# angelvillar96/STLPose

Hardware: AMD Instinct MI355X
Metric: images/sec/GPU HRNet-W32 384x288 train step; PCKh@0.5 parity (higher is better)
Workload: dtype f16/bf16; 1 GPU; HRNet-W32 384x288 bs=32/GPU train step (fwd+MSE+bwd+Adam), random-init weights; global_batch=32, parallelism=dp1

## Files before the change

stlpose_amd/csrc/conv1x1.inc:

```
template <typename T, int G, bool Q, int OCC, typename TY = T, int EO = -1, bool ZM = false>
__global__ __launch_bounds__(512, OCC) void conv1x1_kernel(const ConvK k) {
    extern __shared__ __attribute__((aligned(16))) char smem[];
    constexpr int NTHR = 512, WM = 4, MT = 4, NTW = 2, BCO = 64, TPX = 256;
    constexpr int KV = ET<T>::KV, CK = ET<T>::CK;
    constexpr int PSG = G * 64 + 32;
    constexpr int VPP = 4 * G;
    constexpr int RPT = NTHR / VPP;
    constexpr int NVA = TPX / RPT;
    constexpr int NVB = BCO / RPT;
    constexpr int GK = G * CK;
    static_assert(NVB >= 1, "filter staging needs at least one vector per thread");
    const stl_conv& p = k.p;
    const int tid = threadIdx.x, lane = tid & 63, wave = tid >> 6, r16 = lane & 15, g = lane >> 4;
    const int wm = wave % WM, wn = wave / WM;
    const int bl = blockIdx.x >> 3;
    const int by = bl % k.ny, lx = bl / k.ny;
    const int n0 = by * BCO;
    const int xcd = blockIdx.x & 7, nx = (gridDim.x >> 3) / k.ny;
    const int P = p.B * p.Ho * p.Wo;

    float* cs = reinterpret_cast<float*>(smem + k.off_cs);
    float* cm = reinterpret_cast<float*>(smem + k.off_cm);
    char* sA = smem + k.off_a;
    char* sB = smem + k.off_b;

    for (int c = tid; c < k.cipad; c += NTHR) {
        float a = 0.f, b = 0.f, cc = 0.f;
        if (c < p.Ci) src_consts(p.src, c, p.Ci, a, b, cc);
        cs[c] = a, cs[k.cipad + c] = b, cs[2 * k.cipad + c] = cc;
    }
    if (p.mask_y) {
        for (int c = tid; c < BCO; c += NTHR) {
            float a = 0.f, b = 0.f, mu = 0.f, rs = 0.f;
            if (n0 + c < p.Co) {
                bn_mean_rstd(p.mask_bn, n0 + c, p.Co, mu, rs);
                bn_affine(p.mask_bn.gamma[n0 + c], p.mask_bn.beta[n0 + c], mu, rs, a, b);
            }
            cm[c] = a, cm[BCO + c] = b, cm[2 * BCO + c] = mu, cm[3 * BCO + c] = rs;
        }
    }

    const int a_part = tid % VPP, a_row = tid / VPP;
    V16 ra[NVA], rq[Q ? NVA : 1], rb[NVB];

    auto issue = [&](int P0, int k0, bool en) {
        const int ch = k0 + a_part * KV;
        const bool chok = en && ch < p.Ci;
#pragma unroll
        for (int i = 0; i < NVA; ++i) {
            const int pix = P0 + a_row + i * RPT;
            const size_t off = (chok && pix < P) ? (size_t)pix * p.Ci + ch : 0;
            ra[i] = ldg16((const char*)p.src.x + off * sizeof(T));
            if (Q) rq[i] = ldg16((const char*)p.src.y + off * sizeof(T));
        }
        if (!k.wres) {
#pragma unroll
            for (int i = 0; i < NVB; ++i) {
                const int n = n0 + a_row + i * RPT;
                const size_t off = (chok && n < p.Co) ? (size_t)n * p.Ci + ch : 0;
                rb[i] = ldg16((const char*)p.w + off * sizeof(T));
            }
        }
    };
    const float relu_lo = p.src.relu ? 0.f : -INFINITY;
    auto write_lds = [&](int P0, int k0) {
        const int ch = k0 + a_part * KV;
        const bool chok = ch < p.Ci;
        const int chc = chok ? ch : 0;
#pragma unroll
        for (int i = 0; i < NVA; ++i) {
            const bool ok = chok && (P0 + a_row + i * RPT) < P;
            V16 val = ra[i];
            if constexpr (ZM) {
                val = xform_bnadd<T>(val, rq[i], cs + chc, cs + k.cipad + chc, relu_lo);
                if (ok && by == 0 && p.src_out) stg16((char*)p.src_out + ((size_t)(P0 + a_row + i * RPT) * p.Ci + ch) * sizeof(T), val);
            } else if (Q)
                val = xform_bnbwd<T, TY>(val, rq[i], cs + chc, cs + k.cipad + chc, cs + 2 * k.cipad + chc);
            else if (p.src.mode != STL_SRC_PLAIN)
                val = xform_bn<T>(val, cs + chc, cs + k.cipad + chc, relu_lo);
            mask16(val, ok);
            *reinterpret_cast<V16*>(sA + (a_row + i * RPT) * PSG + a_part * 16) = val;
        }
        if (!k.wres) {
#pragma unroll
            for (int i = 0; i < NVB; ++i) {
                V16 val = rb[i];
                mask16(val, chok && (n0 + a_row + i * RPT) < p.Co);
                *reinterpret_cast<V16*>(sB + (a_row + i * RPT) * PSG + a_part * 16) = val;
            }
        }
    };

    if (k.wres) {
        const bool chok = a_part * KV < p.Ci;
#pragma unroll
        for (int i = 0; i < NVB; ++i) {
            const int n = n0 + a_row + i * RPT;
            const size_t off = (chok && n < p.Co) ? (size_t)n * p.Ci + a_part * KV : 0;
            rb[i] = ldg16((const char*)p.w + off * sizeof(T));
        }
    }

    f2v s0[NTW][2], s1[NTW][2];
#pragma unroll
    for (int ni = 0; ni < NTW; ++ni)
#pragma unroll
        for (int h = 0; h < 2; ++h) s0[ni][h] = f2v{0.f, 0.f}, s1[ni][h] = f2v{0.f, 0.f};
    f32x4 acc[MT][NTW];
#pragma unroll
    for (int mi = 0; mi < MT; ++mi)
#pragma unroll
        for (int ni = 0; ni < NTW; ++ni) acc[mi][ni] = f32x4{0.f, 0.f, 0.f, 0.f};

    int xoff[MT];
#pragma unroll
    for (int mi = 0; mi < MT; ++mi) xoff[mi] = ((wm * MT + mi) * 16 + r16) * PSG + g * 16;
    const int woff = (wn * NTW * 16 + r16) * PSG + g * 16;

    const int T8 = (k.npt + 7) >> 3;
    int it = lx, t = xcd * T8 + it, ch0 = 0;
    bool have = (it < T8) && (t < k.npt);
    issue(t * TPX, 0, have);
    if (k.wres) {
        const bool chok = a_part * KV < p.Ci;
#pragma unroll
        for (int i = 0; i < NVB; ++i) {
            V16 val = rb[i];
            mask16(val, chok && (n0 + a_row + i * RPT) < p.Co);
            *reinterpret_cast<V16*>(sB + (a_row + i * RPT) * PSG + a_part * 16) = val;
        }
    }
    __syncthreads();

    while (have) {
        const int P0 = t * TPX;
        write_lds(P0, ch0 * GK);
        __syncthreads();
        const bool last_chunk = (ch0 + 1 == k.nchunks);
        int itn = it, tn = t, chn = ch0 + 1;
        bool have_n = true;
        if (last_chunk) {
            itn = it + nx, tn = xcd * T8 + itn, chn = 0;
            have_n = (itn < T8) && (tn < k.npt);
        }
        issue(tn * TPX, chn * GK, have_n);
#pragma unroll
        for (int sub = 0; sub < G; ++sub) {
            V16 wf[NTW], xf[MT];
#pragma unroll
            for (int ni = 0; ni < NTW; ++ni) wf[ni] = *reinterpret_cast<const V16*>(sB + woff + ni * 16 * PSG + sub * 64);
#pragma unroll
            for (int mi = 0; mi < MT; ++mi) xf[mi] = *reinterpret_cast<const V16*>(sA + xoff[mi] + sub * 64);
#pragma unroll
            for (int mi = 0; mi < MT; ++mi)
#pragma unroll
                for (int ni = 0; ni < NTW; ++ni) mma16<T>(acc[mi][ni], wf[ni], xf[mi]);
        }
        __syncthreads();
        if (last_chunk) {
#pragma unroll
            for (int mi = 0; mi < MT; ++mi) {
                const int pix = P0 + (wm * MT + mi) * 16 + r16;
                const bool pok = pix < P;
                epilogue_tile<T, NTW, BCO, false, TY, EO>(p, acc[mi], cm, pok, pok ? (size_t)pix * p.Co : 0, n0, wn * NTW * 16, g, s0, s1);
            }
        }
        it = itn, t = tn, ch0 = chn, have = have_n;
    }
    double* dst = p.out_stats ? p.out_stats : p.red;
    if (dst) {
        xor_reduce_stats<NTW>(s0, s1);
        float* red = reinterpret_cast<float*>(smem + k.off_red);
        __syncthreads();
        if (r16 == 0) {
#pragma unroll
            for (int ni = 0; ni < NTW; ++ni)
#pragma unroll
                for (int r = 0; r < 4; ++r) {
                    const int cl = (wn * NTW + ni) * 16 + 4 * g + r;
                    red[(wm * 2 + 0) * BCO + cl] = s0[ni][r >> 1][r & 1];
                    red[(wm * 2 + 1) * BCO + cl] = s1[ni][r >> 1][r & 1];
                }
        }
        __syncthreads();
        for (int e = tid; e < 2 * BCO; e += NTHR) {
            const int which = e / BCO, cl = e - which * BCO;
            float s = 0.f;
#pragma unroll
            for (int w = 0; w < WM; ++w) s += red[(w * 2 + which) * BCO + cl];
            if (n0 + cl < p.Co)
                atomicAdd(dst + (size_t)(blockIdx.x & (STL_NSHARD - 1)) * 2 * p.Co + which * p.Co + n0 + cl, (double)s);
        }
    }
}

template <typename T, typename TY, int G, bool Q, int OCC, int EO = -1, bool ZM = false>
int launch_1x1(const ConvK& k, dim3 grid, size_t lds, hipStream_t st) {
    static bool attr_done = false;
    if (!attr_done) {
        (void)hipFuncSetAttribute(reinterpret_cast<const void*>(&conv1x1_kernel<T, G, Q, OCC, TY, EO, ZM>), hipFuncAttributeMaxDynamicSharedMemorySize,
                                  160 * 1024);
        attr_done = true;
    }
    STL_LAUNCH((conv1x1_kernel<T, G, Q, OCC, TY, EO, ZM>), grid, dim3(512), lds, st, k);
    static char nbuf[160];
    static const char* nm = stl_kname<T>(nbuf, "conv1x1_kernel", {G, Q, OCC, stl_code<TY>(), EO, ZM});
    stl_note_kernel(nm, true);
    STL_LAUNCH_CHECK("conv1x1");
    return 0;
}

static bool use_1x1(const stl_conv& p) { return p.ks == 1 && p.stride == 1 && !p.stuff && p.Ci >= 64 && p.Co >= 64; }

template <typename T, typename TY>
int run_1x1(const stl_conv& p, hipStream_t st) {
    constexpr int CK = ET<T>::CK;
    constexpr int G = 2;
    const int gk = G * CK, psg = G * 64 + 32;
    ConvK k;
    memset(&k, 0, sizeof(k));
    k.p = p;
    k.nchunks = ceil_div(p.Ci, gk);
    k.cipad = k.nchunks * gk;
    k.wres = k.nchunks == 1;
    int off = 3 * k.cipad * 4;
    k.off_cs = 0, k.off_cm = off;
    off += 4 * 64 * 4;
    off = (off + 15) & ~15;
    k.off_a = off;
    off += 256 * psg;
    k.off_b = off;
    off += 64 * psg;
    k.off_red = k.off_a;
    const size_t lds = (size_t)off;
    const int P = p.B * p.Ho * p.Wo;
    k.npt = ceil_div(P, 256);
    k.ny = ceil_div(p.Co, 64);
    int gx = ceil_div(k.npt, 8) * 8;
    int cap = std::max(8, (512 / k.ny + 7) / 8 * 8);
    if (const char* e = getenv("STL_CONV_GRID_CAP")) cap = atoi(e) > 0 ? (atoi(e) + 7) / 8 * 8 : cap;
    if (gx > cap) gx = cap;
    dim3 grid(gx * k.ny, 1);
    if (getenv("STL_CONV_DEBUG"))
        fprintf(stderr, "[stl conv1x1] %dx%d Ci%d Co%d: G=%d npt=%d grid=(%d x %d) lds=%zu nchunks=%d\n", p.Ho, p.Wo, p.Ci, p.Co, G, k.npt, gx,
                k.ny, lds, k.nchunks);
    if (p.src.mode == STL_SRC_BNADD) {
        if constexpr (std::is_same<T, TY>::value) {
            const int eoz = epi_code(p);
            if (eoz == 8) return launch_1x1<T, T, 2, true, 4, 8, true>(k, grid, lds, st);
            if (eoz == 0) return launch_1x1<T, T, 2, true, 4, 0, true>(k, grid, lds, st);
        }
        return stl_set_error("conv1x1: a BNADD source takes no epilogue operands");
    }
    const bool q = p.src.mode == STL_SRC_BNBWD;
    const char* noeo = getenv("STL_CONV_NO_EO");
    const int eo = (noeo && (atoi(noeo) & 2)) ? -1 : epi_code(p);
    if (q) {
        if constexpr (!stl_fwd_only<T>) {
            if (eo == 2) return launch_1x1<T, TY, 2, true, 4, 2>(k, grid, lds, st);
            return launch_1x1<T, TY, 2, true, 4>(k, grid, lds, st);
        }
    }
    if constexpr (std::is_same<T, TY>::value) {
        if (eo == 8) return launch_1x1<T, T, 2, false, 4, 8>(k, grid, lds, st);
        return launch_1x1<T, T, 2, false, 4>(k, grid, lds, st);
    }
    return stl_set_error("conv1x1: no kernel for this dtype combination");
}
```

stlpose_amd/csrc/conv_core.hip:

```cpp
#include <stdlib.h>
#include <algorithm>
#include <cstring>
#include <type_traits>
#include "common.cuh"

#ifndef STL_DT
#define STL_DT 2
#endif
#define STL_HAS_F32 (STL_DT == 0 || STL_DT == 2)
#define STL_HAS_BF16 (STL_DT == 1 || STL_DT == 2)
#define STL_HAS_F16 (STL_DT == 3 || STL_DT == 2)
#define STL_HAS_F32S (STL_DT == 4 || STL_DT == 2)

struct ConvK {
    stl_conv p;
    int tiles_c, npt;
    int HR, HC, HP;
    int PI, pad, seff;
    int nchunks, wres;
    int cipad;
    int off_cs, off_cm, off_a, off_b, off_red;
    int sz_a, sz_b;
    int TH, TW;
    int dbg;
// ... 242 lines not shown
    const int T8 = (k.npt + 7) >> 3;
    const int vpitch = p.Ho + 1;

    int it_n = lx, t_n = xcd * T8 + lx, ch_n = 0;
    bool have_n = (it_n < T8) && (t_n < k.npt);
    auto prefetch = [&]() __attribute__((always_inline)) {
        if (have_n && ch_n == 0) tile_setup(t_n, a_go);
        st_t = t_n, st_ch = ch_n, st_have = have_n;
        issue(a_go, ch_n * CK, have_n);
        if (++ch_n == k.nchunks) {
            ch_n = 0, it_n += nx, t_n = xcd * T8 + it_n;
            have_n = have_n && (it_n < T8) && (t_n < k.npt);
        }
    };
    STAMP(3);
    if constexpr (!DB) {
        prefetch();
        if (wres) {
#pragma unroll
            for (int i = 0; i < NVB; ++i) {
                const bool ok = b_g[i] >= 0 && (((tid + i * NTHR) & 3) * KV) < p.Ci;
                V16 val = rb[i];
                mask16(val, ok);
                if (tid + i * NTHR < BCO * TAPS * 4) *reinterpret_cast<V16*>(sB + b_l[i]) = val;
            }
        }
        __syncthreads();
    }
    STAMP(4);

    f32x4 acc[MT][NTW];
#pragma unroll
    for (int mi = 0; mi < MT; ++mi)
#pragma unroll
        for (int ni = 0; ni < NTW; ++ni) acc[mi][ni] = f32x4{0.f, 0.f, 0.f, 0.f};

    constexpr bool EPRE = (OCC <= 1 && WM == 4 && WN == 2 && NTW == 2) && Q && !PE && !ZM && sizeof(T) == 2;
    constexpr bool EBURST = !EPRE && (EO == 1 || EO == 2) && !PE && sizeof(T) == 2;
    auto out_pixel = [&](int vr0, int c0, int mi, bool& pok) __attribute__((always_inline)) -> size_t {
        const int eb0 = sdiv(vr0, k.m_vp), ey0 = vr0 - eb0 * vpitch;
        int eyx = e_yx[mi];
        if constexpr (DB) {
            const int m = (wm * MT + mi) * 16 + r16, ty_ = fdiv(m, k.r_TW);
            eyx = m < tilepx ? ((ty_ << 16) | (m - ty_ * k.TW)) : -1;
        }
        const int ty = eyx >> 16, tx = eyx & 0xffff;
        const int oy0 = ey0 + ty, c = c0 + tx;
        const int wr_ = fdiv(oy0, k.r_vp);
        const int oy = mad24_vsv(wr_, -vpitch, oy0), b = eb0 + wr_;
        pok = (eyx >= 0) & (b < p.B) & (oy < p.Ho) & (c < p.Wo);
        const int e = mulu24_vs(madu24_vsv(madu24_vsv(b, p.Ho, oy), p.Wo, c), p.Co);
        return pok ? (size_t)(uint32_t)e : 0;
    };
    auto epi_fetch = [&](int vr0, int c0, bool* pokv, size_t* pixv, EpiRaw<NTW>* er) __attribute__((always_inline)) {
#pragma unroll
        for (int mi = 0; mi < MT; ++mi) {
            pixv[mi] = out_pixel(vr0, c0, mi, pokv[mi]);
            epilogue_fetch<T, NTW, true, EO>(p, pokv[mi], pixv[mi], n0, wn * NTW * 16, g, er[mi]);
        }
    };

    if constexpr (DB) {
        constexpr int NSLOT = NVA + NVB;
        prefetch();
        int cu_t = st_t, cu_ch = st_ch;
        bool cu_have = st_have;
        __syncthreads();
        write_lds(a_go, st_ch * CK);
        prefetch();
        __syncthreads();
        int img = 0;
        [[maybe_unused]] int dbg_it = 0;
        while (cu_have) {
            STAMP2(4 * dbg_it);
            const int t = cu_t, ch0 = cu_ch;
            const int tr = sdiv(t, k.m_tc), tc = t - tr * k.tiles_c;
            const int vr0 = tr * k.TH, c0 = tc * k.TW;
            const bool last_chunk = (ch0 + 1 == k.nchunks);
            bool pokv[EPRE ? MT : 1];
            size_t pixv[EPRE ? MT : 1];
            EpiRaw<NTW> er[EPRE ? MT : 1];
            const int k0w = st_ch * CK, k0n = ch_n * CK;
            const bool en_n = have_n, nt = have_n && ch_n == 0;
            int y0n = 0, cbn = 0, b0n = 0;
            if (nt) tile_terms(t_n, y0n, cbn, b0n);
            constexpr bool KREG = !Q || EO == 0 || EO == 1 || EO == 2;
            constexpr int NPK = sizeof(T) == 2 ? 4 : 2;
            f2v kca[NPK], kcb[NPK], kcc[Q ? NPK : 1];
            if constexpr (KREG) {
                const int ch = k0w + a_part * KV;
#pragma unroll
                for (int i = 0; i < NPK; ++i) {
                    kca[i] = reinterpret_cast<const f2v*>(cs + ch)[i];
                    kcb[i] = reinterpret_cast<const f2v*>(cs + k.cipad + ch)[i];
                    if (Q) kcc[i] = reinterpret_cast<const f2v*>(cs + 2 * k.cipad + ch)[i];
                }
            }
            const char* sAr = sA + img * k.sz_a;
            const char* sBr = sB + img * k.sz_b;
            char* sAw = sA + (img ^ 1) * k.sz_a;
            char* sBw = sB + (img ^ 1) * k.sz_b;
            auto slot = [&](int j) __attribute__((always_inline)) {
                if (j < NVA) {
                    const int i = j;
                    const int ch = k0w + a_part * KV;
                    const bool ok = a_go[i] >= 0 && ch < p.Ci;
                    V16 val = ra[i];
                    if constexpr (KREG) {
                        if (Q)
                            val = xform_bnbwd_r<T, TY>(val, rq[i], kca, kcb, kcc);
                        else if (p.src.mode != STL_SRC_PLAIN)
                            val = xform_bn_r<T>(val, kca, kcb, relu_lo);
                    } else {
                        val = xform_bnbwd<T, TY>(val, rq[i], cs + ch, cs + k.cipad + ch, cs + 2 * k.cipad + ch);
                    }
                    mask16(val, ok);
                    int v = tid + i * NTHR;
                    asm volatile("" : "+v"(v));
                    if (v < k.HP * 4) *reinterpret_cast<V16*>(sAw + (v >> 2) * PSA + (v & 3) * 16) = val;
                    if (nt) {
                        const int hp = v >> 2, hr = fdiv(hp, k.r_HC);
                        a_go[i] = slot_go(v < k.HP * 4 ? ((hr << 16) | (hp - hr * k.HC)) : -1, y0n, cbn, b0n);
                    }
                    const bool chok = en_n && (k0n + a_part * KV) < p.Ci;
                    const int off = (a_go[i] >= 0 && chok) ? a_go[i] + k0n : 0;
                    ra[i] = ldg16((const char*)p.src.x + (size_t)(uint32_t)off * sizeof(T));
                    if (Q) rq[i] = ldg16((const char*)p.src.y + (size_t)(uint32_t)off * sizeof(T));
                } else {
                    const int i = j - NVA;
                    int v = tid + i * NTHR;
                    asm volatile("" : "+v"(v));
                    const int part = (v & 3) * KV;
                    const int n = mulu24_vs(v, 1821) >> 16;
                    const bool vok = (i + 1) * NTHR <= BCO * TAPS * 4 || v < BCO * TAPS * 4;
                    const bool rok = vok && n0 + n < p.Co;
                    const int bg = madu24_vsv((v >> 2) + n0 * TAPS, p.Ci, part);
                    V16 val = rb[i];
                    mask16(val, rok && (k0w + part) < p.Ci);
                    if (vok) *reinterpret_cast<V16*>(sBw + v * 16 + n * 32) = val;
                    const bool okn = en_n && rok && (k0n + part) < p.Ci;
                    rb[i] = ldg16((const char*)p.w + (size_t)(uint32_t)(okn ? bg + k0n : 0) * sizeof(T));
                }
            };
            {
                V16 wf[2][NTW], xf[2][MT];
#pragma unroll
                for (int ni = 0; ni < NTW; ++ni) wf[0][ni] = *reinterpret_cast<const V16*>(sBr + woff + ni * 16 * ROWB);
#pragma unroll
                for (int mi = 0; mi < MT; ++mi) xf[0][mi] = *reinterpret_cast<const V16*>(sAr + xoff[mi]);
#pragma unroll
                for (int tap = 0; tap < TAPS; ++tap) {
                    if (tap + 1 < TAPS) {
                        const int toff = (((tap + 1) / KS) * k.HC + ((tap + 1) % KS)) * PSA;
#pragma unroll
                        for (int ni = 0; ni < NTW; ++ni)
                            wf[(tap + 1) & 1][ni] = *reinterpret_cast<const V16*>(sBr + woff + ni * 16 * ROWB + (tap + 1) * 64);
#pragma unroll
                        for (int mi = 0; mi < MT; ++mi) xf[(tap + 1) & 1][mi] = *reinterpret_cast<const V16*>(sAr + xoff[mi] + toff);
                    }
                    __builtin_amdgcn_sched_barrier(0);
#pragma unroll
                    for (int mi = 0; mi < MT; ++mi)
#pragma unroll
                        for (int ni = 0; ni < NTW; ++ni) mma16<T>(acc[mi][ni], wf[tap & 1][ni], xf[tap & 1][mi]);
#pragma unroll
                    for (int j = tap; j < NSLOT; j += TAPS) slot(j);
                    if constexpr (EPRE) {
                        if (tap == (NVA < TAPS ? NVA : TAPS - 1) && last_chunk) epi_fetch(vr0, c0, pokv, pixv, er);
                    }
                    __builtin_amdgcn_sched_barrier(0);
                }
            }
            cu_t = st_t, cu_ch = st_ch, cu_have = st_have;
            st_t = t_n, st_ch = ch_n, st_have = have_n;
            if (++ch_n == k.nchunks) {
                ch_n = 0, it_n += nx, t_n = xcd * T8 + it_n;
                have_n = have_n && (it_n < T8) && (t_n < k.npt);
            }
            STAMP2(4 * dbg_it + 1);
            __syncthreads();
            STAMP2(4 * dbg_it + 2);
            img ^= 1;
            if (last_chunk) {
                if constexpr (EPRE) {
#pragma unroll
                    for (int mi = 0; mi < MT; ++mi)
                        epilogue_apply<T, NTW, BCO, false, TY, EO>(p, acc[mi], cm, pokv[mi], pixv[mi], n0, wn * NTW * 16, g, s0, s1, er[mi]);
                } else {
#pragma unroll
                    for (int mi = 0; mi < MT; ++mi) {
                        bool pok;
                        const size_t pix = out_pixel(vr0, c0, mi, pok);
                        epilogue_tile<T, NTW, BCO, PE, TY, EO>(p, acc[mi], cm, pok, pix, n0, wn * NTW * 16, g, s0, s1);
                    }
                }
            }
            STAMP2(4 * dbg_it + 3);
#ifdef STL_STAMPS
            ++dbg_it;
#endif
        }
    } else
    while (st_have) {
        const int t = st_t, ch0 = st_ch;
        const int tr = sdiv(t, k.m_tc), tc = t - tr * k.tiles_c;
        const int vr0 = tr * k.TH, c0 = tc * k.TW;
        write_lds(a_go, ch0 * CK);
        __syncthreads();
        if (ch0 == 0) STAMP(5);
        const bool last_chunk = (ch0 + 1 == k.nchunks);
        bool pokv[EPRE ? MT : 1];
        size_t pixv[EPRE ? MT : 1];
        EpiRaw<NTW> er[EPRE ? MT : 1];
        if constexpr (EPRE) {
            if (last_chunk) epi_fetch(vr0, c0, pokv, pixv, er);
        }
        prefetch();
        if (ch0 == 0) STAMP(6);
        {
            constexpr bool PIN = (STL_PIN_TAPS != 0);
            V16 wf[2][NTW], xf[2][MT];
#pragma unroll
            for (int ni = 0; ni < NTW; ++ni) wf[0][ni] = *reinterpret_cast<const V16*>(sB + woff + ni * 16 * ROWB);
#pragma unroll
            for (int mi = 0; mi < MT; ++mi) xf[0][mi] = *reinterpret_cast<const V16*>(sA + xoff[mi]);
#pragma unroll
            for (int tap = 0; tap < TAPS; ++tap) {
                if (tap + 1 < TAPS) {
                    const int toff = (((tap + 1) / KS) * k.HC + ((tap + 1) % KS)) * PSA;
#pragma unroll
                    for (int ni = 0; ni < NTW; ++ni)
                        wf[(tap + 1) & 1][ni] = *reinterpret_cast<const V16*>(sB + woff + ni * 16 * ROWB + (tap + 1) * 64);
#pragma unroll
                    for (int mi = 0; mi < MT; ++mi) xf[(tap + 1) & 1][mi] = *reinterpret_cast<const V16*>(sA + xoff[mi] + toff);
                }
                if constexpr (PIN) __builtin_amdgcn_sched_barrier(0);
#pragma unroll
                for (int mi = 0; mi < MT; ++mi)
#pragma unroll
                    for (int ni = 0; ni < NTW; ++ni) mma16<T>(acc[mi][ni], wf[tap & 1][ni], xf[tap & 1][mi]);
                if constexpr (PIN) __builtin_amdgcn_sched_barrier(0);
            }
        }
        __syncthreads();
        if (ch0 == 0) STAMP(7);
        if (last_chunk) {
            STAMP(8);
            if constexpr (EPRE) {
#pragma unroll
                for (int mi = 0; mi < MT; ++mi)
                    epilogue_apply<T, NTW, BCO, false, TY, EO>(p, acc[mi], cm, pokv[mi], pixv[mi], n0, wn * NTW * 16, g, s0, s1, er[mi]);
            } else if constexpr (EBURST) {
                bool pokb[MT];
                size_t pixb[MT];
                EpiRaw<NTW> erb[MT];
                epi_fetch(vr0, c0, pokb, pixb, erb);
#pragma unroll
                for (int mi = 0; mi < MT; ++mi)
                    epilogue_apply<T, NTW, BCO, false, TY, EO>(p, acc[mi], cm, pokb[mi], pixb[mi], n0, wn * NTW * 16, g, s0, s1, erb[mi]);
            } else {
#pragma unroll
                for (int mi = 0; mi < MT; ++mi) {
                    bool pok;
                    const size_t pix = out_pixel(vr0, c0, mi, pok);
                    epilogue_tile<T, NTW, BCO, PE, TY, EO>(p, acc[mi], cm, pok, pix, n0, wn * NTW * 16, g, s0, s1);
                }
            }
        }
        if (last_chunk) STAMP(9);
    }
    STAMP(10);
    double* dst = p.out_stats ? p.out_stats : p.red;
    if (dst) {
        xor_reduce_stats<NTW>(s0, s1);
        float* red = reinterpret_cast<float*>(smem + k.off_red);
        __syncthreads();
        if (r16 == 0) {
#pragma unroll
            for (int ni = 0; ni < NTW; ++ni)
#pragma unroll
                for (int r = 0; r < 4; ++r) {
                    const int cl = (wn * NTW + ni) * 16 + 4 * g + r;
                    red[(wm * 2 + 0) * BCO + cl] = s0[ni][r >> 1][r & 1];
                    red[(wm * 2 + 1) * BCO + cl] = s1[ni][r >> 1][r & 1];
                }
        }
        __syncthreads();
        for (int e = tid; e < 2 * BCO; e += NTHR) {
            const int which = e / BCO, cl = e - which * BCO;
            float s = 0.f;
#pragma unroll
            for (int w = 0; w < WM; ++w) s += red[(w * 2 + which) * BCO + cl];
            if (n0 + cl < p.Co)
                atomicAdd(dst + (size_t)(blockIdx.x & (STL_NSHARD - 1)) * 2 * p.Co + which * p.Co + n0 + cl, (double)s);
        }
    }
    STAMP(11);
#ifdef STL_STAMPS
    if (k.dbg && blockIdx.x == 0 && blockIdx.y == 0 && threadIdx.x == 0) g_stamps[13] = __builtin_amdgcn_s_memtime();
#endif
}

#include "conv_ws.inc"
#include "conv1x1.inc"
#include "conv_r2.inc"

template <typename T, typename TY, int KS, int WM, int WN, int MT, int NTW, int NVA, bool Q, bool PE, int OCC = 1, int WR = -1, bool ZM = false, bool DB = false, int EO = -1>
int launch(const ConvK& k, dim3 grid, size_t lds, hipStream_t st) {
    static bool attr_done = false;
    if (!attr_done) {
        (void)hipFuncSetAttribute(reinterpret_cast<const void*>(&conv_core_kernel<T, KS, WM, WN, MT, NTW, NVA, Q, PE, OCC, WR, ZM, TY, DB, EO>),
                                  hipFuncAttributeMaxDynamicSharedMemorySize, 160 * 1024);
        attr_done = true;
    }
    STL_LAUNCH((conv_core_kernel<T, KS, WM, WN, MT, NTW, NVA, Q, PE, OCC, WR, ZM, TY, DB, EO>), grid, dim3(64 * WM * WN), lds, st, k);
    static char nbuf[160];
    static const char* nm = stl_kname<T>(nbuf, "conv_core_kernel", {KS, WM, WN, MT, NTW, NVA, Q, PE, OCC, WR, ZM, stl_code<TY>(), DB, EO});
    stl_note_kernel(nm, true);
    STL_LAUNCH_CHECK("conv_core");
    return 0;
}

struct Shape {
    int px, co, thr;
    int ws;
    int lthr, nva_max;
};
constexpr int NSHAPES = 11;
constexpr Shape SHAPES[NSHAPES] = {{128, 64, 256, 0, 256, 9}, {512, 32, 512, 0, 512, 6}, {256, 64, 512, 0, 512, 3},
                                   {256, 64, 512, 2, 512, 3}, {128, 32, 256, 0, 256, 6},
                                   {256, 64, 512, 3, 512, 3}, {128, 64, 512, 3, 512, 2}, {128, 64, 512, 1, 256, 9},
                                   {256, 32, 512, 0, 512, 3}, {128, 32, 512, 1, 256, 3}, {256, 32, 512, 3, 512, 3}};

template <typename T, typename TY, int KS, bool Q, bool PE, int EO = -1>
int dispatch(int shape, int nva, const ConvK& k, dim3 grid, size_t lds, hipStream_t st) {
    constexpr int EOC = (KS == 3 && (Q || EO == 48)) ? EO : -1;
    constexpr int EOW = (KS == 3 && EO != 48) ? EO : -1;
    constexpr int OCC4 = (Q || (std::is_same<T, f32s>::value && KS == 3 && !PE)) ? 3 : 4;
    switch (shape) {
        case 0:
            if (nva <= 3) return launch<T, TY, KS, 4, 1, 2, 4, 3, Q, PE>(k, grid, lds, st);
            if (nva <= 9) return launch<T, TY, KS, 4, 1, 2, 4, 9, Q, PE>(k, grid, lds, st);
            break;
        case 1:
            if (nva <= 6) return launch<T, TY, KS, 8, 1, 4, 2, 6, Q, PE>(k, grid, lds, st);
            break;
        case 2:
            if (nva <= 3) return launch<T, TY, KS, 4, 2, 4, 2, 3, Q, PE, 1>(k, grid, lds, st);
            break;
        case 3:
            if constexpr (KS == 3) {
                if (nva <= 3 && !k.wres) return launch<T, TY, KS, 4, 2, 4, 2, 3, Q, PE, 1, 0, false, true, EOC>(k, grid, lds, st);
            }
            break;
        case 8:
            if (nva <= 3 && k.wres) return launch<T, TY, KS, 8, 1, 2, 2, 3, Q, PE, 4, 1, false, false, EOC>(k, grid, lds, st);
            if (nva <= 3) return launch<T, TY, KS, 8, 1, 2, 2, 3, Q, PE, OCC4>(k, grid, lds, st);
            break;
        case 4:
            if (nva <= 3 && k.wres) return launch<T, TY, KS, 4, 1, 2, 2, 3, Q, PE, 4, 1>(k, grid, lds, st);
            if (nva <= 3) return launch<T, TY, KS, 4, 1, 2, 2, 3, Q, PE, OCC4>(k, grid, lds, st);
            if (nva <= 6) return launch<T, TY, KS, 4, 1, 2, 2, 6, Q, PE, 3>(k, grid, lds, st);
            break;
        case 7:
            if (nva <= 3) return launch_ws<T, TY, KS, 2, 4, 3, Q, (Q ? -1 : EOW)>(k, grid, lds, st);
            if (nva <= 9) return launch_ws<T, TY, KS, 2, 4, 9, Q, (Q ? -1 : EOW)>(k, grid, lds, st);
            break;
        case 9:
            if (nva <= 3) return launch_ws<T, TY, KS, 2, 2, 3, Q, EOW>(k, grid, lds, st);
            break;
    }
    return stl_set_error("conv: no kernel variant for block shape %d with %d staging vectors per thread", shape, nva);
}

static bool bnadd_shape_ok(int shape, int nva) { return nva <= 3 && (shape == 0 || shape == 2 || shape == 3 || shape == 4 || shape == 5 || shape == 6 || shape == 8 || shape == 10); }
template <typename T>
int dispatch_bnadd(int shape, int nva, const ConvK& k, dim3 grid, size_t lds, hipStream_t st) {
    if (nva <= 3) switch (shape) {
        case 0: return launch<T, T, 3, 4, 1, 2, 4, 3, true, true, 1, -1, true>(k, grid, lds, st);
        case 2:
        case 3: return launch<T, T, 3, 4, 2, 4, 2, 3, true, true, 1, -1, true>(k, grid, lds, st);
        case 4: return launch<T, T, 3, 4, 1, 2, 2, 3, true, true, 3, -1, true>(k, grid, lds, st);
        case 8: return launch<T, T, 3, 8, 1, 2, 2, 3, true, true, 3, -1, true>(k, grid, lds, st);
    }
    return stl_set_error("conv: no block-end (BNADD) variant for block shape %d with %d staging vectors per thread", shape, nva);
}

template <typename T, typename TY>
int conv_backend(int path, const stl_conv& p, const ConvK& k, int shape, int nva, dim3 grid, size_t lds, hipStream_t st) {
    const bool q = p.src.mode == STL_SRC_BNBWD;
    if constexpr (!std::is_same<T, TY>::value) {
        if (!q) return stl_set_error("conv: ydtype differs from dtype, but the launch is not a data gradient (BNBWD source)");
    }
    if constexpr (std::is_same<T, f16>::value) {
        if (q) return stl_set_error("conv: STL_F16 is a forward-tensor type; gradients are bf16 (dtype STL_BF16 + ydtype STL_F16)");
    }
    if constexpr (std::is_same<T, f32s>::value) {
        if (q) return stl_set_error("conv: math = STL_MATH_BF16X3 has no data-gradient (BNBWD source) kernels");
    }
    constexpr bool FWD = std::is_same<T, TY>::value, BWD = !stl_fwd_only<T>;
    if (path == 0) return run_1x1<T, TY>(p, st);
    if (path == 3) {
        if constexpr (sizeof(T) == 2) return dispatch_r2<T, TY>(p, k, shape == 5 ? 0 : (shape == 6 ? 1 : 2), grid, lds, st);
        return stl_set_error("conv_r2: 16-bit element types only");
    }
    if (path == 1) {
        if constexpr (FWD) return dispatch_bnadd<T>(shape, nva, k, grid, lds, st);
    }
    const bool plain = !p.bias && !p.addend && !p.mask_y && !p.mask_z && !p.red;
    const char* noeo = getenv("STL_CONV_NO_EO");
    const int eo = (noeo && (atoi(noeo) & 1)) ? -1 : epi_code(p);
    if (p.ks == 3) {
        if (q) {
            if constexpr (BWD) {
                if (eo == 1) return dispatch<T, TY, 3, true, false, 1>(shape, nva, k, grid, lds, st);
                if (eo == 7) return dispatch<T, TY, 3, true, false, 7>(shape, nva, k, grid, lds, st);
                if (eo == 2) return dispatch<T, TY, 3, true, false, 2>(shape, nva, k, grid, lds, st);
                if (eo == 0) return dispatch<T, TY, 3, true, false, 0>(shape, nva, k, grid, lds, st);
                return dispatch<T, TY, 3, true, false>(shape, nva, k, grid, lds, st);
            }
        }
        if constexpr (FWD) {
            if (plain && eo == 8) return dispatch<T, T, 3, false, true, 8>(shape, nva, k, grid, lds, st);
            if (!plain && eo == 48) return dispatch<T, T, 3, false, false, 48>(shape, nva, k, grid, lds, st);
            return plain ? dispatch<T, T, 3, false, true>(shape, nva, k, grid, lds, st) : dispatch<T, T, 3, false, false>(shape, nva, k, grid, lds, st);
        }
    }
    if (q) {
        if constexpr (BWD) return dispatch<T, TY, 1, true, false>(shape, nva, k, grid, lds, st);
    }
    if constexpr (FWD) return plain ? dispatch<T, T, 1, false, true>(shape, nva, k, grid, lds, st) : dispatch<T, T, 1, false, false>(shape, nva, k, grid, lds, st);
    return stl_set_error("conv: no kernel for this dtype combination");
}

struct Plan {
    int shape, TH, TW;
    size_t lds;
    double cost;
};

size_t lds_bytes(const stl_conv& p, int shape, int TH, int TW, int ck, ConvK* out) {
    const int taps = p.ks * p.ks, seff = p.stride;
    const int HR = (TH - 1) * seff + p.ks, HC = (TW - 1) * seff + p.ks;
    const int nchunks = ceil_div(p.Ci, ck), cipad = nchunks * ck;
    const int bco = SHAPES[shape].co, ws = SHAPES[shape].ws;
    if (ws == 3) {
        int off = 3 * cipad * 4;
        const int off_cm = off;
        off = (off + 4 * bco * 4 + 15) & ~15;
        const int off_a = off, pl = ((HR * HC * R2_PS) + 15) & ~15;
        off += 2 * pl;
        const int off_b = (off + 1023) & ~1023;
        off = off_b + bco * R2_ROWF;
        const int off_red = off;
        off += 512 * 4;
        if (out) {
            out->HR = HR, out->HC = HC, out->HP = HR * HC, out->nchunks = nchunks, out->cipad = cipad;
            out->off_cs = 0, out->off_cm = off_cm, out->off_a = off_a, out->off_b = off_b, out->off_red = off_red;
            out->sz_a = pl, out->sz_b = 0, out->wres = 0;
        }
        return (size_t)off;
    }
    int off = 3 * cipad * 4;
    const int off_cm = off;
    off += 4 * bco * 4;
    off = (off + 15) & ~15;
    const int off_a = off;
    const int sz_a = ((HR * HC * PSA) + 15) & ~15;
    off += sz_a * (ws ? 2 : 1);
    const int off_b = off;
    const int sz_b = bco * (taps * 64 + 32);
    const bool resident = nchunks == 1 || (ws == 1 && (size_t)off + (size_t)sz_b * nchunks <= 150 * 1024);
    off += resident ? sz_b * nchunks : sz_b * (ws ? 2 : 1);
    const int off_red = off_a;
    const int red = 8 * 2 * bco * 4;
    if (off - off_a < red) off = off_a + red;
    if (out) {
        out->HR = HR, out->HC = HC, out->HP = HR * HC, out->nchunks = nchunks, out->cipad = cipad;
        out->off_cs = 0, out->off_cm = off_cm, out->off_a = off_a, out->off_b = off_b, out->off_red = off_red;
        out->sz_a = ws ? sz_a : 0, out->sz_b = (ws && !resident) ? sz_b : 0;
        out->wres = resident ? 1 : 0;
    }
    return (size_t)off;
}

Plan choose_plan(const stl_conv& p, int ck) {
    Plan best{-1, 0, 0, 0, 1e300};
    const int vrows = p.B * (p.Ho + 1);
    const int r2_env = getenv("STL_CONV_R2") ? atoi(getenv("STL_CONV_R2")) : 11;
    const bool deep_small = p.stride == 1 && p.ks == 3 && p.Co >= 256 && (int64_t)p.B * p.Ho * p.Wo <= 16384 &&
                            !((r2_env & 8) && p.dtype != STL_F32 && p.Ci % 32 == 0 && p.Ci >= 64 && (r2_env & (p.src.mode == STL_SRC_BNBWD ? 2 : 1)));
    const bool want_ws = p.stride == 2 || deep_small;
    const bool wide_k = p.Co <= 32 && p.Ci >= 128 && p.stride == 1 && p.ks == 3 && !p.stuff && (int64_t)p.B * p.Ho * p.Wo >= 65536;
    const bool c32 = p.Co <= 32 && p.stride == 1 && p.ks == 3 && !wide_k;
    for (int shape = 0; shape < NSHAPES; ++shape) {
        const Shape sh = SHAPES[shape];
        if (sh.px == 0) continue;
        if (sh.px > 128 && p.stride == 2) continue;
        if ((sh.ws == 1) != want_ws) continue;
        if (want_ws && shape != (deep_small ? 9 : 7)) continue;
        if (shape == 2 || shape == 3 || shape == 5 || shape == 6) {
            static const bool db_on = !(getenv("STL_CONV_DB") && atoi(getenv("STL_CONV_DB")) == 0);
            const int r2_mode = r2_env;
            const bool db = db_on && p.ks == 3 && p.stride == 1 && p.Ci > ck;
            const bool dgrad = p.src.mode == STL_SRC_BNBWD;
            const bool r2 = db && (r2_mode & (dgrad ? 2 : 1)) && p.dtype != STL_F32 && p.Ci % 32 == 0 && p.Ci >= 64;
            const bool small_map = (r2_mode & 8) && p.Co >= 256 && (int64_t)p.B * p.Ho * p.Wo <= 16384;
            const int want = r2 ? ((dgrad || (r2_mode & 4) || small_map) ? 6 : 5) : (db ? 3 : 2);
            if (shape != want) continue;
        }
        if ((shape == 1 || shape == 8 || shape == 10) && p.Co > 32) continue;
        if ((shape == 4 || shape == 8 || shape == 10) && !c32) continue;
        if (c32 && shape != 4 && shape != 8 && shape != 10) continue;
        {
            const bool r2c32 = (r2_env & 16) && p.dtype != STL_F32 && p.Ci == 32 && (r2_env & (p.src.mode == STL_SRC_BNBWD ? 2 : 1));
            if (c32 && (shape == 8 || shape == 10) && (shape == 10) != r2c32) continue;
        }
        if (wide_k && shape != 1) continue;
        const int nblk_co = ceil_div(p.Co, sh.co);
        for (int tw = (p.Wo < 4 ? p.Wo : 4); tw <= p.Wo && tw <= sh.px; ++tw)
          for (int frac = 4; frac >= 1; --frac) {
            int th = (sh.px / tw) * frac / 4;
            if (th > vrows) th = vrows;
            if (th < 1) continue;
            const int hr = (th - 1) * p.stride + p.ks, hc = (tw - 1) * p.stride + p.ks;
            const int nva = ceil_div(hr * hc * 4, sh.lthr);
            if (nva > sh.nva_max) continue;
            const size_t lds = lds_bytes(p, shape, th, tw, ck, nullptr);
            if (shape == 4 && lds > 40 * 1024 && nva <= 3) continue;
            if (shape == 8 && lds > 80 * 1024) continue;
            if ((shape == 5 || shape == 6 || shape == 10) && lds > 76 * 1024) continue;
            if (lds > 158 * 1024) continue;
            const double tiles = (double)ceil_div(vrows, th) * ceil_div(p.Wo, tw);
            const double mfma = tiles * sh.px * sh.co * nblk_co * (double)p.Ci * p.ks * p.ks / 2048.0;
            const double bytes = tiles * nblk_co * ((double)hr * hc * p.Ci + (double)sh.co * p.ks * p.ks * p.Ci) * 2.0 / 12.0;
            const double blocks = tiles * nblk_co;
            double cost = (mfma > bytes ? mfma : bytes) + 0.3 * (mfma < bytes ? mfma : bytes);
            const double waves = blocks * sh.thr / 64.0;
            if (waves < 2048.0) cost *= 1.0 + 0.15 * (2048.0 / waves - 1.0 > 4.0 ? 4.0 : 2048.0 / waves - 1.0);
            if (c32 && shape == 4) cost *= 4.0;
            if (shape == 5 || shape == 6 || shape == 10) cost *= 0.98;
            if (cost < best.cost) best = Plan{shape, th, tw, lds, cost};
        }
    }
    return best;
}

}

#if STL_HAS_BF16
static bool math_ok(const stl_conv& p) {
    return p.math == STL_MATH_NATIVE || (p.math == STL_MATH_BF16X3 && p.dtype == STL_F32 && p.src.mode != STL_SRC_BNBWD && !p.stuff);
}
static const char* math_error(const stl_conv& p, const char* who) {
    static thread_local char buf[200];
    if (p.math != STL_MATH_BF16X3) snprintf(buf, sizeof(buf), "%s: math %d (STL_MATH_NATIVE or STL_MATH_BF16X3)", who, p.math);
    else if (p.dtype != STL_F32) snprintf(buf, sizeof(buf), "%s: math = STL_MATH_BF16X3 needs dtype STL_F32 (got dtype %d)", who, p.dtype);
    else if (p.stuff) snprintf(buf, sizeof(buf), "%s: math = STL_MATH_BF16X3 does not go with stuff = 1 (a data gradient)", who);
    else snprintf(buf, sizeof(buf), "%s: math = STL_MATH_BF16X3 does not go with a BNBWD source (src.mode, a data gradient)", who);
    return buf;
}
static int ydtype_of(const stl_conv& p) { return (p.dtype == STL_BF16 && p.ydtype == STL_F16) ? STL_F16 : p.dtype; }
int stl_conv_backend_bf16(int path, const stl_conv& p, const ConvK& k, int shape, int nva, dim3 grid, size_t lds, hipStream_t st) {
    if (ydtype_of(p) == STL_F16) return conv_backend<__bf16, f16>(path, p, k, shape, nva, grid, lds, st);
    return conv_backend<__bf16, __bf16>(path, p, k, shape, nva, grid, lds, st);
}
#endif
#if STL_HAS_F32
int stl_conv_backend_f32(int path, const stl_conv& p, const ConvK& k, int shape, int nva, dim3 grid, size_t lds, hipStream_t st) {
    return conv_backend<float, float>(path, p, k, shape, nva, grid, lds, st);
}
#endif
#if STL_HAS_F16
int stl_conv_backend_f16(int path, const stl_conv& p, const ConvK& k, int shape, int nva, dim3 grid, size_t lds, hipStream_t st) {
    return conv_backend<f16, f16>(path, p, k, shape, nva, grid, lds, st);
}
#endif
#if STL_HAS_F32S
int stl_conv_backend_f32s(int path, const stl_conv& p, const ConvK& k, int shape, int nva, dim3 grid, size_t lds, hipStream_t st) {
    return conv_backend<f32s, f32s>(path, p, k, shape, nva, grid, lds, st);
}
#endif

#if STL_HAS_BF16
#ifdef STL_STAMPS
extern "C" int stl_debug_conv_stamps(long long* host12) {
    return hipMemcpyFromSymbol(host12, HIP_SYMBOL(g_stamps), 14 * sizeof(long long)) == hipSuccess ? 0 : stl_set_error("stamps: copy failed");
}
extern "C" int stl_debug_conv_stamps2(long long* host64) {
    return hipMemcpyFromSymbol(host64, HIP_SYMBOL(g_stamps2), 64 * sizeof(long long)) == hipSuccess ? 0 : stl_set_error("stamps: copy failed");
}
#endif

extern "C" int stl_conv_plan(stl_conv* pp) {
    stl_conv& p = *pp;
    STL_CHECK(p.dtype == STL_F32 || p.dtype == STL_BF16 || p.dtype == STL_F16, "conv_plan: bad dtype");
    STL_CHECK((p.ks == 1 || p.ks == 3) && (p.stride == 1 || p.stride == 2) && p.Ci > 0 && p.Co > 0, "conv_plan: bad geometry");
    STL_CHECK(math_ok(p), "%s", math_error(p, "conv_plan"));
    const int ck = p.dtype == STL_F32 ? 16 : 32;
    Plan plan = choose_plan(p, ck);
    STL_CHECK(plan.shape >= 0, "conv_plan: no tile fits LDS for %dx%d ks %d stride %d Ci %d", p.Ho, p.Wo, p.ks, p.stride, p.Ci);
    p.shape = plan.shape, p.TH = plan.TH, p.TW = plan.TW;
    return 0;
}

extern "C" int stl_conv_bnadd_ok(const stl_conv* pp) {
// ... 112 lines not shown
```

Before: 2512 images/sec.

## Add streaming 1x1 conv kernel with register-prefetched activations for 16-bit types

```diff
diff --git a/stlpose_amd/csrc/conv1x1.inc b/stlpose_amd/csrc/conv1x1.inc
--- a/stlpose_amd/csrc/conv1x1.inc
+++ b/stlpose_amd/csrc/conv1x1.inc
@@ -214,6 +214,7 @@
 
 template <typename T, typename TY>
 int run_1x1(const stl_conv& p, hipStream_t st) {
+    if (stream_1x1_takes<T, TY>(p)) return run_1x1s<T, TY>(p, st);
     constexpr int CK = ET<T>::CK;
     constexpr int G = 2;
     const int gk = G * CK, psg = G * 64 + 32;
diff --git a/stlpose_amd/csrc/conv1x1s.inc b/stlpose_amd/csrc/conv1x1s.inc
--- /dev/null
+++ b/stlpose_amd/csrc/conv1x1s.inc
@@ -0,0 +1,264 @@
+constexpr int occ_1x1s(int EO) { return (EO & 1) ? 3 : 4; }
+
+template <typename T, typename TY, int NST, int MODE, int EO>
+__global__ __launch_bounds__(256, occ_1x1s(EO)) void conv1x1s_kernel(const ConvK k) {
+    extern __shared__ __attribute__((aligned(16))) char smem[];
+    constexpr int NTHR = 256, NW = 4, NTW = 4, BCO = 64, CI = NST * 64;
+    constexpr int PSG = CI * 2 + 32;
+    constexpr bool Q = MODE == STL_SRC_BNBWD;
+    constexpr int D = (Q && (EO & 1)) ? 1 : 2;
+    constexpr bool EP = !(NST == 4 && EO == 7);
+    static_assert(sizeof(T) == 2 && sizeof(TY) == 2, "16-bit element types only");
+    const stl_conv& p = k.p;
+    const int tid = threadIdx.x, lane = tid & 63, r16 = lane & 15, g = lane >> 4;
+    const int wave = __builtin_amdgcn_readfirstlane(tid >> 6);
+    const int bl = blockIdx.x >> 3;
+    const int by = bl % k.ny, lx = bl / k.ny;
+    const int n0 = by * BCO;
+    const int xcd = blockIdx.x & 7, nx = (gridDim.x >> 3) / k.ny;
+    const int P = p.B * p.Ho * p.Wo;
+
+    float* cs = reinterpret_cast<float*>(smem);
+    float* cm = reinterpret_cast<float*>(smem + 3 * CI * 4);
+    char* sB = smem + 3 * CI * 4 + 4 * BCO * 4;
+
+    const int T8 = (k.npt + 7) >> 3, step = nx * NW;
+    int it = lx * NW + wave;
+    auto tile_ok = [&](int i) { return i < T8 && xcd * T8 + i < k.npt; };
+    auto src_off = [&](int i) {
+        const int pix = (xcd * T8 + i) * 16 + r16;
+        return (tile_ok(i) && pix < P) ? (uint32_t)(pix * CI + 8 * g) * 2u : (uint32_t)(16 * g);
+    };
+    auto out_pix = [&](int i, bool& pok) {
+        const int pix = (xcd * T8 + i) * 16 + r16;
+        pok = tile_ok(i) && pix < P;
+        return pok ? (size_t)pix * p.Co : 0;
+    };
+    V16 rx[D][2], ry[Q ? D : 1][2];
+    uint32_t o[3] = {src_off(it), src_off(it + step), src_off(it + 2 * step)};
+    auto issue = [&](int d, int ahead) __attribute__((always_inline)) {
+        const uint32_t oo = o[ahead / NST] + (ahead % NST) * 128;
+#pragma unroll
+        for (int j = 0; j < 2; ++j) {
+            rx[d][j] = ldg16((const char*)p.src.x + oo + j * 64);
+            if constexpr (Q) ry[d][j] = ldg16((const char*)p.src.y + oo + j * 64);
+        }
+    };
+#pragma unroll
+    for (int d = 0; d < D; ++d) issue(d, d);
+    EpiRaw<2> e[2], en[2];
+    bool pok;
+    size_t po = out_pix(it, pok);
+    if constexpr (EP) {
+        epilogue_fetch<T, 2, false, EO>(p, pok, po, n0, 0, g, e[0]);
+        epilogue_fetch<T, 2, false, EO>(p, pok, po, n0, 32, g, e[1]);
+    }
+
+    if constexpr (MODE != STL_SRC_PLAIN) {
+        for (int c = tid; c < CI; c += NTHR) {
+            float a, b, cc;
+            src_consts(p.src, c, CI, a, b, cc);
+            cs[c] = a, cs[CI + c] = b, cs[2 * CI + c] = cc;
+        }
+    }
+    if constexpr (EO >= 0 && (EO & 1)) {
+        for (int c = tid; c < BCO; c += NTHR) {
+            float a, b, mu, rs;
+            bn_mean_rstd(p.mask_bn, n0 + c, p.Co, mu, rs);
+            bn_affine(p.mask_bn.gamma[n0 + c], p.mask_bn.beta[n0 + c], mu, rs, a, b);
+            cm[c] = a, cm[BCO + c] = b, cm[2 * BCO + c] = mu, cm[3 * BCO + c] = rs;
+        }
+    }
+    {
+        constexpr int NVB = BCO * (CI / 8) / NTHR;
+        V16 rb[NVB];
+#pragma unroll
+        for (int i = 0; i < NVB; ++i) {
+            const int v = tid + i * NTHR;
+            rb[i] = ldg16((const char*)p.w + ((size_t)(n0 + v / (CI / 8)) * CI + v % (CI / 8) * 8) * 2);
+        }
+#pragma unroll
+        for (int i = 0; i < NVB; ++i) {
+            const int v = tid + i * NTHR;
+            *reinterpret_cast<V16*>(sB + v / (CI / 8) * PSG + v % (CI / 8) * 16) = rb[i];
+        }
+    }
+    __syncthreads();
+
+    f2v s0[NTW][2], s1[NTW][2];
+    f32x4 acc[NTW];
+#pragma unroll
+    for (int ni = 0; ni < NTW; ++ni) {
+        acc[ni] = f32x4{0.f, 0.f, 0.f, 0.f};
+#pragma unroll
+        for (int h = 0; h < 2; ++h) s0[ni][h] = f2v{0.f, 0.f}, s1[ni][h] = f2v{0.f, 0.f};
+    }
+    [[maybe_unused]] const float relu_lo = p.src.relu ? 0.f : -INFINITY;
+    const char* wl = sB + r16 * PSG + g * 16;
+    const float* cl = cs + 8 * g;
+
+    bool have = tile_ok(it);
+    while (have) {
+        const int itn = it + step;
+        int ge = g;
+        asm volatile("" : "+v"(ge));
+        bool pok_n;
+        const size_t po_n = out_pix(itn, pok_n);
+        if constexpr (EO & 7) {
+            epilogue_fetch<T, 2, false, EO>(p, EP ? pok_n : pok, EP ? po_n : po, n0, 0, ge, EP ? en[0] : e[0]);
+            epilogue_fetch<T, 2, false, EO>(p, EP ? pok_n : pok, EP ? po_n : po, n0, 32, ge, EP ? en[1] : e[1]);
+            __builtin_amdgcn_sched_barrier(0);
+        }
+#pragma unroll
+        for (int st = 0; st < NST; ++st) {
+            asm volatile("" ::: "memory");
+            __builtin_amdgcn_sched_barrier(0);
+            V16 xv[2];
+#pragma unroll
+            for (int j = 0; j < 2; ++j) {
+                const int s = st * 2 + j;
+                if constexpr (MODE == STL_SRC_PLAIN) {
+                    xv[j] = rx[0][j];
+                } else {
+                    f2v ca[4], cb[4];
+#pragma unroll
+                    for (int i = 0; i < 4; ++i) {
+                        ca[i] = *reinterpret_cast<const f2v*>(cl + s * 32 + 2 * i);
+                        cb[i] = *reinterpret_cast<const f2v*>(cl + CI + s * 32 + 2 * i);
+                    }
+                    if constexpr (Q) {
+                        f2v cc[4];
+#pragma unroll
+                        for (int i = 0; i < 4; ++i) cc[i] = *reinterpret_cast<const f2v*>(cl + 2 * CI + s * 32 + 2 * i);
+                        xv[j] = xform_bnbwd_r<T, TY>(rx[0][j], ry[0][j], ca, cb, cc);
+                    } else {
+                        xv[j] = xform_bn_r<T>(rx[0][j], ca, cb, relu_lo);
+                    }
+                }
+            }
+#pragma unroll
+            for (int d = 0; d + 1 < D; ++d)
+#pragma unroll
+                for (int j = 0; j < 2; ++j) {
+                    rx[d][j] = rx[d + 1][j];
+                    if constexpr (Q) ry[d][j] = ry[d + 1][j];
+                }
+            issue(D - 1, st + D);
+#pragma unroll
+            for (int j = 0; j < 2; ++j)
+#pragma unroll
+                for (int ni = 0; ni < NTW; ++ni) {
+                    const V16 wf = *reinterpret_cast<const V16*>(wl + ni * 16 * PSG + (st * 2 + j) * 64);
+                    mma16<T>(acc[ni], wf, xv[j]);
+                }
+        }
+        epilogue_apply<T, 2, BCO, false, TY, EO>(p, acc, cm, pok, po, n0, 0, ge, s0, s1, e[0]);
+        asm volatile("" ::: "memory");
+        epilogue_apply<T, 2, BCO, false, TY, EO>(p, acc + 2, cm, pok, po, n0, 32, ge, s0 + 2, s1 + 2, e[1]);
+        it = itn, have = tile_ok(it), pok = pok_n, po = po_n;
+        if constexpr (EP) e[0] = en[0], e[1] = en[1];
+        o[0] = o[1], o[1] = o[2], o[2] = src_off(it + 2 * step);
+    }
+
+    if constexpr (EO >= 0 && (EO & 9)) {
+        double* dst = (EO & 8) ? p.out_stats : p.red;
+        xor_reduce_stats<NTW>(s0, s1);
+        float* red = reinterpret_cast<float*>(sB);
+        __syncthreads();
+        if (r16 == 0) {
+#pragma unroll
+            for (int ni = 0; ni < NTW; ++ni)
+#pragma unroll
+                for (int r = 0; r < 4; ++r) {
+                    const int c = ni * 16 + 4 * g + r;
+                    red[(wave * 2 + 0) * BCO + c] = s0[ni][r >> 1][r & 1];
+                    red[(wave * 2 + 1) * BCO + c] = s1[ni][r >> 1][r & 1];
+                }
+        }
+        __syncthreads();
+        for (int e = tid; e < 2 * BCO; e += NTHR) {
+            const int which = e / BCO, c = e - which * BCO;
+            float s = 0.f;
+#pragma unroll
+            for (int w = 0; w < NW; ++w) s += red[(w * 2 + which) * BCO + c];
+            atomicAdd(dst + (size_t)(blockIdx.x & (STL_NSHARD - 1)) * 2 * p.Co + which * p.Co + n0 + c, (double)s);
+        }
+    }
+}
+
+template <typename T, typename TY, int NST, int MODE, int EO>
+int launch_1x1s(const ConvK& k, dim3 grid, size_t lds, hipStream_t st) {
+    STL_LAUNCH((conv1x1s_kernel<T, TY, NST, MODE, EO>), grid, dim3(256), lds, st, k);
+    static char nbuf[160];
+    static const char* nm = stl_kname<T>(nbuf, "conv1x1s_kernel", {stl_code<TY>(), NST, MODE, EO});
+    stl_note_kernel(nm, true);
+    STL_LAUNCH_CHECK("conv1x1s");
+    return 0;
+}
+
+constexpr int STL_1X1S_MIN_PIXELS = 65536;
+
+template <typename T, typename TY>
+bool stream_1x1_takes(const stl_conv& p) {
+    if constexpr (sizeof(T) != 2) return false;
+    const char* e = getenv("STL_CONV1X1_STREAM");
+    const int sw = e ? atoi(e) : -1;
+    if (sw == 0) return false;
+    if (p.ks != 1 || p.stride != 1 || p.stuff) return false;
+    if ((p.Ci != 64 && p.Ci != 256) || p.Co % 64 != 0) return false;
+    const int eo = epi_code(p);
+    bool faster = false;
+    if (p.src.mode == STL_SRC_BNBWD) {
+        if (stl_fwd_only<T> || !(eo == 0 || eo == 1 || eo == 2 || eo == 7)) return false;
+        faster = p.Ci == 256 ? (eo == 0 || eo == 1) : eo == 7;
+    } else if (p.src.mode == STL_SRC_PLAIN || p.src.mode == STL_SRC_BN) {
+        if (!std::is_same<T, TY>::value || !(eo == 0 || eo == 8)) return false;
+    } else {
+        return false;
+    }
+    return sw == 1 || (faster && (int64_t)p.B * p.Ho * p.Wo >= STL_1X1S_MIN_PIXELS);
+}
+
+template <typename T, typename TY, int NST, int MODE>
+int run_1x1s_eo(const ConvK& k, int eo, dim3 grid, size_t lds, hipStream_t st) {
+    if constexpr (MODE == STL_SRC_BNBWD) {
+        if (eo == 1) return launch_1x1s<T, TY, NST, MODE, 1>(k, grid, lds, st);
+        if (eo == 2) return launch_1x1s<T, TY, NST, MODE, 2>(k, grid, lds, st);
+        if (eo == 7) return launch_1x1s<T, TY, NST, MODE, 7>(k, grid, lds, st);
+        return launch_1x1s<T, TY, NST, MODE, 0>(k, grid, lds, st);
+    } else {
+        if (eo == 8) return launch_1x1s<T, TY, NST, MODE, 8>(k, grid, lds, st);
+        return launch_1x1s<T, TY, NST, MODE, 0>(k, grid, lds, st);
+    }
+}
+
+template <typename T, typename TY>
+int run_1x1s(const stl_conv& p, hipStream_t st) {
+    if constexpr (sizeof(T) == 2) {
+        ConvK k;
+        memset(&k, 0, sizeof(k));
+        k.p = p;
+        const size_t lds = 3 * p.Ci * 4 + 4 * 64 * 4 + 64 * (p.Ci * 2 + 32);
+        const int P = p.B * p.Ho * p.Wo;
+        k.npt = ceil_div(P, 16);
+        k.ny = p.Co / 64;
+        int gx = ceil_div(ceil_div(k.npt, 4), 8) * 8;
+        const int eo = epi_code(p);
+        int cap = std::max(8, (256 * occ_1x1s(eo) / k.ny + 7) / 8 * 8);
+        if (const char* e = getenv("STL_CONV_GRID_CAP")) cap = atoi(e) > 0 ? (atoi(e) + 7) / 8 * 8 : cap;
+        if (gx > cap) gx = cap;
+        dim3 grid(gx * k.ny, 1);
+        if (getenv("STL_CONV_DEBUG"))
+            fprintf(stderr, "[stl conv1x1s] %dx%d Ci%d Co%d: npt=%d grid=(%d x %d) lds=%zu\n", p.Ho, p.Wo, p.Ci, p.Co, k.npt, gx, k.ny, lds);
+        const bool wide = p.Ci == 256;
+        if (p.src.mode == STL_SRC_BNBWD) {
+            if constexpr (!stl_fwd_only<T>)
+                return wide ? run_1x1s_eo<T, TY, 4, STL_SRC_BNBWD>(k, eo, grid, lds, st) : run_1x1s_eo<T, TY, 1, STL_SRC_BNBWD>(k, eo, grid, lds, st);
+        } else if constexpr (std::is_same<T, TY>::value) {
+            if (p.src.mode == STL_SRC_BN)
+                return wide ? run_1x1s_eo<T, T, 4, STL_SRC_BN>(k, eo, grid, lds, st) : run_1x1s_eo<T, T, 1, STL_SRC_BN>(k, eo, grid, lds, st);
+            return wide ? run_1x1s_eo<T, T, 4, STL_SRC_PLAIN>(k, eo, grid, lds, st) : run_1x1s_eo<T, T, 1, STL_SRC_PLAIN>(k, eo, grid, lds, st);
+        }
+    }
+    return stl_set_error("conv1x1s: no kernel for this launch");
+}
diff --git a/stlpose_amd/csrc/conv_core.hip b/stlpose_amd/csrc/conv_core.hip
--- a/stlpose_amd/csrc/conv_core.hip
+++ b/stlpose_amd/csrc/conv_core.hip
@@ -568,6 +568,7 @@
 }
 
 #include "conv_ws.inc"
+#include "conv1x1s.inc"
 #include "conv1x1.inc"
 #include "conv_r2.inc"
 
```

Result: no change. 2492 images/sec (-0.8%).
